# davide-coccomini/MINTIME-Multi-Identity-size-iNvariant-TIMEsformer-for-Video-Deepfake-Detection

Hardware: AMD Instinct MI355X
Metric: clips/sec (8-frame, 2-identity, 224^2 crops) fwd+bwd (higher is better)
Workload: dtype f32; 1 GPU; config 3: EfficientNet-B0 + SizeInvariantTimeSformer(dim 512, depth 9, heads 8), B=32/GPU, 8 frames, 2 identities (identity-masked), 224x224 crops, random-init seeded weights (restored before every step), train-mode BN + drop-connect 0.2, step = fwd + BCE loss + bwd + SGD(lr .01, wd 1e-4); global_batch=32, frames=8, parallelism=dp1

## Files before the change

include/mintime_hip.h:

```cpp
#ifndef MINTIME_HIP_H
#define MINTIME_HIP_H
#include <stdint.h>
#ifdef __cplusplus
extern "C" {
#endif

#define MT_VERSION 123

int mt_version(void);
const char* mt_last_error(void);

int mt_set_deterministic(int on);
int mt_get_deterministic(void);
int mt_det_release(void* stream);
int mt_det_bn_sums(const float* x, const float* z, const float* mean_invstd, int64_t rows, int C, int mode, double* stats, void* stream);

typedef struct { int gin, gout, off; } mt_rowmap;

enum { MT_OP_NT = 0,
       MT_OP_NN = 1,
       MT_OP_TN = 2 };

enum { MT_PRO_NONE = 0, MT_PRO_BN_SWISH_GATE = 1, MT_PRO_BN_SWISH = 2, MT_PRO_AFFINE = 3,
       MT_PRO_BN_BWD = 4,
// ... 48 lines not shown

int mt_bn_bwd_apply_planes(const float* du, const float* z, const float* kabc, void* planes, int rows, int C, void* stream);

typedef struct {
  int op;
  int epilogue;
  int M, N, K;
  const void* a_planes;
  const void* b_planes;
  float* C; int64_t ldc;
  const float* bias;
  const float* R; int64_t ldr;
  float* C2; int64_t ldc2;
  int n_half;
  float* col_sum;
  void* c_planes;
  int split_k;
  void* sk_workspace;
  int64_t sk_workspace_bytes;
  double* stats; int stats_slots;
} mt_gemm_planes_desc;

int mt_gemm_planes(const mt_gemm_planes_desc* d, void* stream);

int mt_mul_planes(const float* x, const float* m, void* planes, float* out, int rows, int cols, void* stream);
int mt_mul_add(const float* y, const float* m, const float* r, float* out, int64_t n, void* stream);
int mt_geglu_bwd(const float* dh, const float* m, const float* u, void* du_planes, float* du, int rows, int n_half, void* stream);
int64_t mt_gemm_planes_workspace_bytes(void);
int mt_gemm_planes_set_persist(int blocks_per_cu);


int mt_layernorm_fwd(const float* x, const float* gamma, const float* beta, float* y, float* stats,
                     int rows, int dim, float eps, void* y_planes, void* stream);

int mt_embed_fwd(float* x, const float* cls, const float* pos_emb, const float* size_emb,
                 const int64_t* positions, const int32_t* sizes, int B, int F, int n, int dim, int pos_rows, int size_rows,
                 int* err_flag, void* stream);

int mt_attn_fwd(const float* qkv, float* out, float* cls_att, const uint8_t* mask, const uint8_t* ident,
                int B, int H, int F, int n, int mode, float scale, void* out_planes, void* stream);

int mt_head_fwd(const float* x, const float* gamma, const float* beta, const float* w, const float* bias,
                float* logits, int B, int N, int dim, int classes, float eps, void* stream);


int mt_stem_conv_fwd(const void* x, int x_is_u8, const float* w, float* z, double* stats, int slots, int N, int H, int W,
// ... 256 lines not shown
```

mintime-multi-identity-size-invariant-timesformer-for-video-deepfake-detection_amd/csrc/gemm_planes.hip:

```cpp
#include "../../include/mintime_hip.h"
#include "common.hpp"
#include "gemm_planes_launch.hpp"
#include "gemm_geometry.hpp"
#include "det.hpp"
#include <string.h>

using namespace mt;

namespace {

__device__ __forceinline__ void to_blk_block(const float* __restrict__ src, int64_t ld, int R, int C, const PlaneRef& o, int rb, int cb, int lane) {
  const int r = rb * 32 + (lane >> 1), c = cb * 16 + (lane & 1) * 8;
  float x[8] = {0.f, 0.f, 0.f, 0.f, 0.f, 0.f, 0.f, 0.f};
  if (r < R) {
    const float* s = src + (int64_t)r * ld + c;
    if (c + 8 <= C && ((ld & 3) == 0) && (((uintptr_t)src & 15) == 0)) {
      const float4 u = *reinterpret_cast<const float4*>(s), v = *reinterpret_cast<const float4*>(s + 4);
      x[0] = u.x; x[1] = u.y; x[2] = u.z; x[3] = u.w; x[4] = v.x; x[5] = v.y; x[6] = v.z; x[7] = v.w;
    } else {
#pragma unroll
      for (int e = 0; e < 8; ++e) if (c + e < C) x[e] = s[e];
    }
  }
  planes_store8(o, r, c, x);
// ... 89 lines not shown
  const int cb16 = (cols + 15) >> 4, rp = (rows + 31) & ~31;
  const PlaneRef o{reinterpret_cast<__bf16*>(planes), (int64_t)rp * cb16 * 16, cb16, rp};
  hipLaunchKernelGGL(split_planes_blk_kernel, dim3((cb16 + 3) / 4, rp / 32), dim3(256), 0, (hipStream_t)stream, src, ld, rows, cols, o);
  return check_launch("mt_split_planes_blk");
}

extern "C" int mt_bn_bwd_apply_planes(const float* du, const float* z, const float* kabc, void* planes, int rows, int C, void* stream) {
  if (!du || !z || !kabc || !planes || rows <= 0 || C <= 0) return fail(MT_ERR_ARG, "mt_bn_bwd_apply_planes: bad arguments");
  if ((C & 3) || (((uintptr_t)du | (uintptr_t)z | (uintptr_t)kabc | (uintptr_t)planes) & 15))
    return fail(MT_ERR_ARG, "mt_bn_bwd_apply_planes: C %% 4 == 0 and 16-byte alignment");
  const int cb16 = (C + 15) >> 4, rp = (rows + 31) & ~31;
  const PlaneRef o{reinterpret_cast<__bf16*>(planes), (int64_t)rp * cb16 * 16, cb16, rp};
  hipLaunchKernelGGL(bn_bwd_apply_planes_kernel, dim3((cb16 + 3) / 4, rp / 32), dim3(256), 0, (hipStream_t)stream, du, z, kabc, rows, C, o);
  return check_launch("mt_bn_bwd_apply_planes");
}

extern "C" int mt_split_planes_blk_multi(const void* items, int count, int64_t total_blocks, void* stream) {
  if (!items || count <= 0 || total_blocks <= 0) return fail(MT_ERR_ARG, "mt_split_planes_blk_multi: bad arguments");
  hipLaunchKernelGGL(split_planes_blk_multi_kernel, dim3((unsigned)((total_blocks + 3) / 4)), dim3(256), 0, (hipStream_t)stream,
                     reinterpret_cast<const SplitItem*>(items), count, total_blocks);
  return check_launch("mt_split_planes_blk_multi");
}

static int gemm_planes_impl(const mt_gemm_planes_desc* d, void* stream) {
  if (!d || !d->a_planes || !d->b_planes) return fail(MT_ERR_ARG, "mt_gemm_planes: null operand planes");
  if (d->M <= 0 || d->N <= 0 || d->K <= 0) return fail(MT_ERR_ARG, "mt_gemm_planes: bad shape %d %d %d", d->M, d->N, d->K);
  if (((uintptr_t)d->a_planes & 15) || ((uintptr_t)d->b_planes & 15) || ((uintptr_t)d->c_planes & 15))
    return fail(MT_ERR_ARG, "mt_gemm_planes: planes must be 16-byte aligned");
  const int op = d->op, epi = d->epilogue;
  const bool cpl = d->c_planes != nullptr;
  if (!d->C && !cpl) return fail(MT_ERR_ARG, "mt_gemm_planes: no output");
  if (cpl && epi != MT_EPI_GEGLU && epi != MT_EPI_GEGLU_BWD) return fail(MT_ERR_UNSUPPORTED, "mt_gemm_planes: plane output only from the GEGLU pair");
  if (epi == MT_EPI_BIAS_RES && !d->R) return fail(MT_ERR_ARG, "mt_gemm_planes: BIAS_RES needs R");
  if (epi == MT_EPI_GEGLU && (d->n_half * 2 != d->N || (d->n_half & 63))) return fail(MT_ERR_ARG, "mt_gemm_planes GEGLU: N must be 2*n_half, n_half %% 64 == 0");
  if (epi == MT_EPI_GEGLU_BWD && (!d->C2 || d->n_half != d->N || (d->n_half & 31)))
    return fail(MT_ERR_ARG, "mt_gemm_planes GEGLU_BWD: needs C2, n_half == N and n_half %% 32 == 0");
  hipStream_t s = (hipStream_t)stream;
  const bool high = matmul_precision() == MT_PRECISION_HIGH;
  const int np = high ? 2 : 3;
  auto launch = [&](int skm, const GemmArgs& ga, dim3 g) {
    return high ? launch_planes_high(op, epi, cpl, skm, ga, g, s) : launch_planes_form<3>(op, epi, cpl, skm, ga, g, s);
  };

  const int a_rows = op == MT_OP_TN ? d->K : d->M, a_cols = op == MT_OP_TN ? d->M : d->K;
  const int b_rows = op == MT_OP_NT ? d->N : d->K, b_cols = op == MT_OP_NT ? d->K : d->N;
  GemmArgs a;
  memset(&a, 0, sizeof(a));
  a.C = d->C; a.M = d->M; a.N = d->N; a.K = d->K; a.ldc = d->ldc;
  a.a_planes = d->a_planes; a.a_pstride = mt_planes_elems(a_rows, a_cols); a.lda = (a_cols + 15) >> 4;
  a.b_planes = d->b_planes; a.b_pstride = mt_planes_elems(b_rows, b_cols); a.ldb = (b_cols + 15) >> 4;
  if (6 * a.a_pstride > 0xFFFFFFFFll || 6 * a.b_pstride > 0xFFFFFFFFll)
    return fail(MT_ERR_UNSUPPORTED, "mt_gemm_planes: an operand's planes span %lld bytes (> 4 GB: 32-bit DMA offsets); use mt_gemm for it (lib.planes_fit)",
                (long long)(6 * (a.a_pstride > a.b_pstride ? a.a_pstride : a.b_pstride)));
  a.bias = d->bias; a.R = d->R; a.ldr = d->ldr; a.C2 = d->C2; a.ldc2 = d->ldc2; a.n_half = d->n_half; a.col_sum = d->col_sum;
  a.hw = 1; a.stats_slots = d->stats_slots != 0 ? d->stats_slots : 1; a.stats = d->stats; a.b_hw = 1; a.e_hw = 1;
  if (epi == MT_EPI_STATS && !d->stats) return fail(MT_ERR_ARG, "mt_gemm_planes: STATS needs stats");
  if (epi == MT_EPI_GEGLU_BWD)
    if (int rc = det_gemm_colsum_setup(a.det, d->M, d->n_half, d->col_sum, s)) return rc;
  if (cpl) {
    const int c_cols = epi == MT_EPI_GEGLU ? d->n_half : 2 * d->n_half;
    a.c_planes = d->c_planes; a.c_pstride = mt_planes_elems(d->M, c_cols); a.ldcp = (c_cols + 15) >> 4;
  }

  const TileGrid tg = tile_grid(d->M, d->N, 128, 128, (int64_t)128 * d->K * 2 * np);
  const int m_tiles = tg.m_tiles, n_tiles = tg.n_tiles;
  if (op == MT_OP_TN) {
    if (epi != MT_EPI_ATOMIC) return fail(MT_ERR_UNSUPPORTED, "mt_gemm_planes TN: ATOMIC epilogue only (C pre-zeroed)");
    static const int target = env_int("MT_WGRAD_BLOCKS", 640);
    const SplitK sk = split_k_ranges(d->K, m_tiles * n_tiles, d->split_k, target, 16, K_XCD);
    a.k_chunk = sk.k_chunk; a.xcd_k = sk.xcd_k;
    if (int rc = det_gemm_setup(a.C, a.ldc, a.det_slab, d->M, d->N, sk.ranges, false, s)) return rc;
    return launch(0, a, dim3(m_tiles * n_tiles, sk.grid_y, 1));
  }
  dim3 grid(tg.grid_x, 1, 1);
  a.group_n = tg.group_n;
  static const int prio = env_int("MT_PLANES_MAIN_PRIO", 0);
  a.wave_prio = prio;
  bool sk = false;
  if (d->sk_workspace && d->sk_workspace_bytes >= mt_gemm_planes_workspace_bytes() && !((uintptr_t)d->sk_workspace & 255)) {
    int g = cu_count() * 2 / 8 * 8;
    if (g > kSkMaxGrid) g = kSkMaxGrid;
    const int64_t units = (int64_t)m_tiles * n_tiles * (((d->K + 15) / 16 + 1) / 2);
    if (g >= 8 && units >= (int64_t)g * 2 && units < (1ll << 30)) {
      sk = true;
      grid = dim3((unsigned)g, 1, 1);
      a.sk_on = 1;
      a.sk_flags = reinterpret_cast<int*>(d->sk_workspace);
      a.sk_ws = reinterpret_cast<float*>(reinterpret_cast<char*>(d->sk_workspace) + kSkFlagBytes);
    }
  }
  if (!sk && !cpl && (epi == MT_EPI_STORE || epi == MT_EPI_BIAS_RES)) {
    const int per_cu = persist_blocks();
    const int g = cu_count() * per_cu / 8 * 8;
    if (per_cu > 0 && g >= 8 && m_tiles * n_tiles > g) {
      const dim3 pg((unsigned)g, 1, 1);
      const bool nt_store = op == MT_OP_NT && epi == MT_EPI_STORE, nt_bias_res = op == MT_OP_NT && epi == MT_EPI_BIAS_RES;
      const bool nn_store = op == MT_OP_NN && epi == MT_EPI_STORE;
      if (nt_store || nt_bias_res || nn_store) return launch(2, a, pg);
    }
  }
  return launch(sk ? 1 : 0, a, grid);
}

extern "C" int mt_gemm_planes(const mt_gemm_planes_desc* d, void* stream) {
  const int rc = gemm_planes_impl(d, stream);
  if (rc) { (void)mt::det_gemm_finish(nullptr, false); return rc; }
  return mt::det_gemm_finish((hipStream_t)stream, true);
}
```

mintime-multi-identity-size-invariant-timesformer-for-video-deepfake-detection_amd/csrc/gemm_planes.hpp:

```cpp
#pragma once
#include "gemm_split.hpp"
#include "planes.hpp"

#ifndef MT_PLANES_ABLATE
#define MT_PLANES_ABLATE 0
#endif
#ifndef MT_PLANES_EPI_ABLATE
#define MT_PLANES_EPI_ABLATE 0
#endif
#ifndef MT_PLANES_PRIO
#define MT_PLANES_PRIO 0
#endif

namespace mt {

typedef short s16x4_t __attribute__((ext_vector_type(4)));
enum : int { BAL_NONE = 0, BAL_PAIR = 1, BAL_PHASE = 2 };

__device__ __forceinline__ void lds_dma16_s(const void* sbase, unsigned voff, unsigned lds_byte_addr) {
  unsigned keep;
  asm volatile("s_mov_b32 %0, m0\n\ts_mov_b32 m0, %3\n\ts_nop 0\n\tglobal_load_lds_dwordx4 %1, %2\n\ts_mov_b32 m0, %0"
               : "=&s"(keep) : "v"(voff), "s"(sbase), "s"(lds_byte_addr) : "memory");
}

// ... 90 lines not shown
        if (MT_PLANES_EPI_ABLATE & 4) { if (da[3] + dg[5] == 123.456f) p.col_sum[0] = 1.f; }
        else if (n0 + wn * TN * 32 + j * 32 < p.N) {
          planes_emit_tile(da, wl, o, mw + i * 32, n0 + wn * TN * 32 + j * 32, p.M, lane);
          planes_emit_tile(dg, wl, o, mw + i * 32, p.n_half + n0 + wn * TN * 32 + j * 32, p.M, lane);
        }
      }
      if (p.col_sum && !(MT_PLANES_EPI_ABLATE & 16)) {
        float t1 = s1[j], t2 = s2[j];
        t1 += __shfl_xor(t1, 32);
        t2 += __shfl_xor(t2, 32);
        if (lane < 32 && nok) {
          if (p.det.vals) {
            const int rk = mw >> 5;
            det_put(p.det, n >> 5, rk, n & 31, t1);
            det_put(p.det, (p.n_half + n) >> 5, rk, n & 31, t2);
            if (rk == 0 && (n & 31) == 0) { det_base(p.det, n >> 5, n); det_base(p.det, (p.n_half + n) >> 5, p.n_half + n); }
          } else {
            atomicAdd(p.col_sum + n, t1);
            atomicAdd(p.col_sum + p.n_half + n, t2);
          }
        }
      }
    }
  }
}

template <int BM, int BN>
__device__ __forceinline__ void sk_tile_coords(const GemmArgs& p, int t, int& mt_, int& nt_) {
  const int n_tiles = (p.N + BN - 1) / BN, m_tiles = (p.M + BM - 1) / BM;
  if (p.group_n > 0) {
    const int q = m_tiles >> 3, r = m_tiles & 7;
    int xcd = 0, base = 0;
    for (; xcd < 7; ++xcd) {
      const int cnt = (q + (xcd < r ? 1 : 0)) * n_tiles;
      if (t < base + cnt) break;
      base += cnt;
    }
    const int rows = q + (xcd < r ? 1 : 0);
    const int row0 = xcd < r ? xcd * (q + 1) : r * (q + 1) + (xcd - r) * q;
    const int idx = t - base;
    const int per_group = rows * p.group_n;
    const int g = idx / per_group;
    const int rem = idx - g * per_group;
    const int groups = (n_tiles + p.group_n - 1) / p.group_n;
    const int gw = (g == groups - 1) ? n_tiles - g * p.group_n : p.group_n;
    const int ml = rem / gw;
// ... 271 lines not shown
#pragma unroll
        for (int j = 0; j < TN; ++j) asm volatile("" : "+v"(acc[i][j]));
    }
  };

  auto epilogue = [&](int mt_, int nt_, int split_idx = -1) {
    if (MT_PLANES_ABLATE & 8) {
      float sacc = 0.f;
#pragma unroll
      for (int i = 0; i < TM; ++i)
#pragma unroll
        for (int j = 0; j < TN; ++j)
#pragma unroll
          for (int r = 0; r < 16; ++r) sacc += acc[i][j][r];
      if (sacc == 123.456f) p.C[0] = sacc;
      return;
    }
    int m0e = mt_ * BM, n0e = nt_ * BN, lane_e = lane;
    asm volatile("" : "+s"(m0e), "+s"(n0e), "+v"(lane_e));
    if constexpr (CPL) {
      static_assert(!CPL || STAGES * STAGE >= NW * 32 * 36 * 4, "the plane epilogue's LDS patches live in the main loop's stages");
      __syncthreads();
      planes_epilogue<TM, TN, EPI>(p, acc, m0e, n0e, wm, wn, lane_e, reinterpret_cast<float*>(smem_pl) + wave * (32 * 36));
    } else {
      gemm_epilogue<TM, TN, EPI>(p, acc, m0e, n0e, wm, wn, lane_e, split_idx);
    }
  };

  if (p.wave_prio == 1) __builtin_amdgcn_s_setprio(1);
  else if (p.wave_prio == 2) __builtin_amdgcn_s_setprio(2);
  else if (p.wave_prio == 3) __builtin_amdgcn_s_setprio(3);
  if (MT_PLANES_PRIO == 1) {
    const unsigned hwid = __builtin_amdgcn_s_getreg((4 << 0) | (0 << 6) | (3 << 11));
    if (__builtin_amdgcn_readfirstlane(hwid) & 1) __builtin_amdgcn_s_setprio(1);
  } else if (MT_PLANES_PRIO == 2) {
    if ((blockIdx.x >> 8) & 1) __builtin_amdgcn_s_setprio(1);
  }

  if constexpr (PS) {
    const int Q = gridDim.x >> 3, xcd = blockIdx.x & 7, q = blockIdx.x >> 3;
    const int n_tiles = (p.N + BN - 1) / BN, m_tiles = (p.M + BM - 1) / BM;
    int base = 0, cnt;
    if (p.group_n > 0) {
      const int qq = m_tiles >> 3, rr = m_tiles & 7;
      for (int i = 0; i < xcd; ++i) base += (qq + (i < rr ? 1 : 0)) * n_tiles;
      cnt = (qq + (xcd < rr ? 1 : 0)) * n_tiles;
// ... 212 lines not shown
```

mintime-multi-identity-size-invariant-timesformer-for-video-deepfake-detection_amd/csrc/gemm_planes_launch.hpp:

```cpp
#pragma once
#include "../../include/mintime_hip.h"
#include "common.hpp"
#include "gemm_planes.hpp"

#ifndef MT_PLANES_HIGH_STAGES
#define MT_PLANES_HIGH_STAGES 3
#endif

namespace mt {

template <int NP, bool AKM, bool BKM, int EPI, int BAL, bool CPL, int SK = 0>
int launch_planes(const GemmArgs& a, dim3 grid, hipStream_t s) {
  constexpr int ST = (NP == 2 && SK != 2) ? MT_PLANES_HIGH_STAGES : 2;
  auto k = gemm_planes_kernel<2, 2, 2, 2, AKM, BKM, EPI, ST, BAL == BAL_PAIR ? 2 : 3, BAL, CPL, SK, NP>;
  constexpr size_t lds = (size_t)ST * NP * (128 + 128) * 32;
  {
    hipError_t e = ensure_dynamic_lds(reinterpret_cast<const void*>(k), lds);
    if (e != hipSuccess) return fail(MT_ERR_LAUNCH, "mt_gemm_planes: cannot reserve %zu B of LDS: %s", lds, hipGetErrorString(e));
  }
  hipLaunchKernelGGL(k, grid, dim3(256), lds, s, a);
  return check_launch("mt_gemm_planes");
}

template <int NP>
int launch_planes_form(int op, int epi, bool cpl, int skm, const GemmArgs& a, dim3 grid, hipStream_t s) {
  if (op == MT_OP_TN && epi == MT_EPI_ATOMIC) return launch_planes<NP, true, true, EPI_ATOMIC, BAL_NONE, false, 0>(a, grid, s);
  if (skm == 2 && !cpl) {
    if (op == MT_OP_NT && epi == MT_EPI_STORE) return launch_planes<NP, false, false, EPI_STORE, BAL_PAIR, false, 2>(a, grid, s);
    if (op == MT_OP_NT && epi == MT_EPI_BIAS_RES) return launch_planes<NP, false, false, EPI_BIAS_RES, BAL_PAIR, false, 2>(a, grid, s);
    if (op == MT_OP_NN && epi == MT_EPI_STORE) return launch_planes<NP, false, true, EPI_STORE, BAL_PAIR, false, 2>(a, grid, s);
  }
  if (skm == 0 || skm == 1) {
#define PL_COMBO(OP, BKM_, EPI_, CPL_)                                                               \
  if (op == OP && epi == EPI_ && cpl == CPL_)                                                        \
    return skm ? launch_planes<NP, false, BKM_, EPI_, BAL_PAIR, CPL_, 1>(a, grid, s)                 \
               : launch_planes<NP, false, BKM_, EPI_, BAL_PAIR, CPL_, 0>(a, grid, s);
    PL_COMBO(MT_OP_NT, false, EPI_STORE, false)
    PL_COMBO(MT_OP_NT, false, EPI_BIAS_RES, false)
    PL_COMBO(MT_OP_NT, false, EPI_STATS, false)
    PL_COMBO(MT_OP_NT, false, EPI_GEGLU, false)
    PL_COMBO(MT_OP_NT, false, EPI_GEGLU, true)
    PL_COMBO(MT_OP_NN, true, EPI_STORE, false)
    PL_COMBO(MT_OP_NN, true, EPI_BIAS_RES, false)
    PL_COMBO(MT_OP_NN, true, EPI_GEGLU_BWD, false)
    PL_COMBO(MT_OP_NN, true, EPI_GEGLU_BWD, true)
#undef PL_COMBO
  }
  return fail(MT_ERR_UNSUPPORTED, "mt_gemm_planes: unsupported op / epilogue %d / %d", op, epi);
}

int launch_planes_high(int op, int epi, bool cpl, int skm, const GemmArgs& a, dim3 grid, hipStream_t s);

}
```

mintime-multi-identity-size-invariant-timesformer-for-video-deepfake-detection_amd/effnet_backward.py:

```python
import torch

from . import arch
from . import lib as L
from .effnet_engine import SLOTS, STREAM_ROWS, _StatsPool
from .lib import _new


FUSED_DW = __import__("os").environ.get("MT_DW_FUSED", "3")


def _splits(rows):
    return max(1, min(64, rows // 1024))


LAST_RUN = {"blocks_run": 0, "wgrad_launches": 0, "stem_run": False}


def effnet_backward(model, params, saved, shape, training, dfeat, need_dx, need_dparams, keep_saved=False, plan=None):
    lib = L.get()
    dev = dfeat.device
    N, H, W = shape
    blocks = model._blocks
    P = list(params)
    pos = 3
# ... 17 lines not shown
    if any(need[:3]):
        lowest = -1
    if need_dx:
        lowest = -1
        need_below = [True] * len(blocks)
        if W > 512:
            raise NotImplementedError("gradient w.r.t. the input crops: mt_stem_conv_dgrad takes crops of at most 512 columns")
    def runs_dw(bi):
        s, ix = blocks[bi].spec, bidx[bi]
        return need[ix["d"]] or need_below[bi] or (s.has_expand and any(need[ix["e"]:ix["e"] + 3]))
    odd = [b.spec.idx for bi, b in enumerate(blocks) if bi >= lowest and b.spec.s == 2 and b.spec.hin % 2 and runs_dw(bi)]
    if odd:
        raise NotImplementedError(f"EfficientNet backward for {H} x {W} crops: the stride-2 depthwise layers of blocks {odd} see odd "
                                  "sizes, which mt_dwconv_bwd does not take")
    grads, flat_grads = L.zero_grads(list(params), with_flat=True)
    dx = None
    run = {"blocks_run": 0, "wgrad_launches": 0, "stem_run": False}
    total_c = arch.STEM_COUT + arch.HEAD_COUT + sum((b.spec.cexp if b.spec.has_expand else 0) + b.spec.cexp + b.spec.cout
                                                    for b in blocks)
    tr = 1 if training else 0
    side = L.SideStream(dev, hold=True)

    det = L.deterministic()
    pool = _StatsPool(dev, total_c, det)
    slots = -SLOTS if det else SLOTS
    fused_dw = "0" if det else FUSED_DW

    def bn_finalize(bnctx, sums, gidx_gamma, d=None, z=None, rows=0):
        kabc = _new(dev, 3, bnctx.C)
        L.mt.bn_bwd_finalize(sums, slots, bnctx.count, P[gidx_gamma], bnctx.mean_invstd, kabc, grads[gidx_gamma], grads[gidx_gamma + 1],
                             bnctx.C, tr)
        return kabc

    def act_bwd(din, z, bnctx, dout, rows, hw, act, gate=None, dpool=None, rowscale=None):
        sums = pool.take(bnctx.C)
        L.mt.bn_act_bwd(din, z, bnctx.scale, bnctx.shift, bnctx.mean_invstd, gate, dpool, rowscale, dout, sums, slots, rows, bnctx.C, hw,
                        act)
        return sums

    def conv1x1_bwd(du, z, kabc, w, x_in, rows, cout, cin, gw_idx, need_dx_in, res=None, b_pro=None, pl=None):
        if pl is not None:
            dz_p = L.planes_empty(rows, cout, dev)
            L.mt.bn_bwd_apply_planes(du, z, kabc, dz_p, rows, cout)
            wdone = False
            if need[gw_idx] and pl.get("x_p") is not None:
                run["wgrad_launches"] += 1
                side.launch(lambda: L.gemm_planes(L.OP_TN, dz_p, pl["x_p"], cout, cin, rows, Cout=grads[gw_idx].view(cout, cin), ldc=cin,
                                                  epilogue=L.EPI_ATOMIC), reads=(dz_p, pl["x_p"]))
                wdone = True
            dx_in = None
            if need_dx_in:
                dx_in = _new(dev, rows, cin)
                if res is not None:
                    L.gemm_planes(L.OP_NN, dz_p, pl["w_p"], rows, cin, cout, Cout=dx_in, ldc=cin, epilogue=L.EPI_BIAS_RES, R=res, ldr=cin)
                else:
                    L.gemm_planes(L.OP_NN, dz_p, pl["w_p"], rows, cin, cout, Cout=dx_in, ldc=cin)
            if wdone or not need[gw_idx]:
                return dx_in
            need_dx_in, keep_dx = False, dx_in
        else:
            keep_dx = None
        kw = {}
        if b_pro is not None:
            kw = dict(b_prologue=L.BPRO_BN_SWISH_GATE, b_scale=b_pro[0], b_shift=b_pro[1], b_gate=b_pro[2], b_hw=b_pro[3])
        reads = (du, z, x_in, kabc) + (tuple(b_pro[:3]) if b_pro is not None else ())
        if (not det and b_pro is None and need[gw_idx] and need_dx_in and rows >= STREAM_ROWS
                and lib.mt_conv1x1_bwd_fused_supported(cout, cin)):
            run["wgrad_launches"] += 1
            dx_in = _new(dev, rows, cin)
            L.mt.conv1x1_bwd_fused(du, kabc, x_in, w, res, dx_in, grads[gw_idx], rows, cout, cin)
            return dx_in
        if not need[gw_idx]:
            pass
        elif rows >= STREAM_ROWS and not det and lib.mt_conv1x1_wgrad_supported(cout, cin):
            run["wgrad_launches"] += 1
            bp = b_pro if b_pro is not None else (None, None, None, 1)
            side.launch(lambda: L.mt.conv1x1_wgrad(du, z, kabc, x_in, bp[0], bp[1], bp[2], bp[3], grads[gw_idx], rows, cout, cin),
# ... 26 lines not shown
    M = N * s_last.hout * s_last.hout
    du_h = _new(dev, M, arch.HEAD_COUT)
    sums = act_bwd(dfeat, hd["z"], hd["bn"], du_h, M, 1, 1)
    kabc = bn_finalize(hd["bn"], sums, ih + 1, du_h, hd["z"], M)
    dy = conv1x1_bwd(du_h, hd["z"], kabc, P[ih], hd["y_in"], M, arch.HEAD_COUT, arch.HEAD_CIN, ih, lowest < len(blocks),
                     pl=dict(w_p=hd["w_p"], x_p=hd["y_p"]) if hd.get("w_p") is not None else None)
    del du_h

    for bi in reversed(range(len(blocks))):
        if bi < lowest:
            break
        run["blocks_run"] += 1
        blk, rec, ix = blocks[bi], saved["blocks"][bi], bidx[bi]
        s = rec["spec"]
        M_in, M_out = N * s.hin * s.hin, N * s.hout * s.hout
        hw = s.hout * s.hout
        dc = rec["dc"]
        dyb = _new(dev, M_out, s.cout) if dc is not None else None
        sums = act_bwd(dy, rec["z_p"], rec["bn_p"], dyb, M_out, hw, 0, rowscale=dc)
        dsrc = dyb if dc is not None else dy
        kabc_p = bn_finalize(rec["bn_p"], sums, ix["p"] + 1, dsrc, rec["z_p"], M_out)
        bn_d = rec["bn_d"]
        b_pro = (bn_d.scale, bn_d.shift, rec["gate"], hw)
        dgate, dpre2, dpooled = _new(dev, N, s.cexp), _new(dev, N, s.cexp), _new(dev, N, s.cexp)
        dhid = _new(dev, N, s.cse)
        se_scr = _new(dev, lib.mt_se_scratch_floats(N, s.cexp, s.cse))
        se = ix["se"]
        def se_part(parts, _da=None, _rec=rec, _bn=bn_d, _se=se, _s=s, _dg=dgate, _dp=dpre2, _dh=dhid, _dpo=dpooled, _hw=hw, _scr=se_scr):
            L.mt.se_bwd(_da, _rec["z_d"], _bn.scale, _bn.shift, _rec["gate"], _rec["hidden"], _rec["pooled"], P[_se], P[_se + 2], _dg, _dp,
                        _dh, _dpo, grads[_se], grads[_se + 1], grads[_se + 2], grads[_se + 3], N, _hw, _s.cexp, _s.cse, parts, _scr)
        if not det and M_out >= STREAM_ROWS and lib.mt_se_stage_fused_supported(s.cout, s.cexp, hw):
            conv1x1_bwd(dsrc, rec["z_p"], kabc_p, P[ix["p"]], rec["z_d"], M_out, s.cout, s.cexp, ix["p"], False, b_pro=b_pro)
            def stage(mode, dg, g_, dpo, mi, out, st_):
                L.mt.se_stage_fused(dsrc, rec["z_p"], kabc_p, P[ix["p"]], rec["z_d"], bn_d.scale, bn_d.shift, mode, dg, g_, dpo, mi, out,
                                    st_, slots, M_out, s.cout, s.cexp, hw)
            L.zero_(dgate)
            stage(0, dgate, None, None, None, None, None)
            se_part(4)
            if any(need[se:se + 4]):
                run["wgrad_launches"] += 1
                side.launch(lambda: se_part(2), reads=(dpre2, dhid, rec["hidden"], rec["pooled"]))
            da = _new(dev, M_out, s.cexp)
            sums = pool.take(s.cexp)
            stage(1, None, rec["gate"], dpooled, bn_d.mean_invstd, da, sums)
        else:
            da = conv1x1_bwd(dsrc, rec["z_p"], kabc_p, P[ix["p"]], rec["z_d"], M_out, s.cout, s.cexp, ix["p"], True, b_pro=b_pro,
                             pl=dict(w_p=rec["wp_p"], x_p=rec["a_p"]) if rec.get("wp_p") is not None else None)
            se_part(1, da)
            if any(need[se:se + 4]):
                run["wgrad_launches"] += 1
                side.launch(lambda: se_part(2), reads=(dpre2, dhid, rec["hidden"], rec["pooled"]))
            sums = act_bwd(da, rec["z_d"], bn_d, da, M_out, hw, 1, gate=rec["gate"], dpool=dpooled)
        kabc_d = bn_finalize(bn_d, sums, ix["d"] + 1, da, rec["z_d"], M_out)
        in_bn = rec["dw_bn"]
        du_in = _new(dev, M_in, s.cexp)
        sums_in = pool.take(s.cexp)
        def dw_part(parts, _da=da, _rec=rec, _kabc=kabc_d, _bn=in_bn, _du_in=du_in, _sums=sums_in, _s=s, _ix=ix):
            L.mt.dwconv_bwd(_da, _rec["z_d"], _kabc, P[_ix["d"]], _rec["dw_in"], _bn.scale, _bn.shift, _bn.mean_invstd, _du_in, _sums,
                            slots, grads[_ix["d"]], N, _s.hin, _s.hin, _s.cexp, _s.k, _s.s, parts, 1, None, None)
        need_du_in = need_below[bi] or (s.has_expand and any(need[ix["e"]:ix["e"] + 3]))
        dw_bytes = 4.0 * s.cexp * (2 * M_out + 2 * M_in)
        if not need_du_in or not need[ix["d"]]:
            if need[ix["d"]]:
                run["wgrad_launches"] += 1
                side.launch(lambda: dw_part(1), reads=(da, rec["z_d"], kabc_d, rec["dw_in"], in_bn.scale, in_bn.shift))
            if need_du_in:
                L.timed("dwconv_dgrad", lambda: dw_part(2), dw_bytes)
        elif fused_dw == "1" or (fused_dw == "3" and s.k == 3):
            run["wgrad_launches"] += 1
            L.timed("dwconv_dgrad", lambda: dw_part(3), dw_bytes)
        else:
# ... 35 lines not shown
```

mintime-multi-identity-size-invariant-timesformer-for-video-deepfake-detection_amd/effnet_engine.py:

```python
import threading

import torch

from . import arch
from . import lib as L
from . import plans
from .lib import _new

SLOTS = 32
STREAM_ROWS = 100000
EF_PLANES_EXPAND_HW, EF_PLANES_PROJECT_HW = 14, 7


def param_list(model):
    ps = [model._conv_stem.weight, model._bn0.weight, model._bn0.bias]
    for blk in model._blocks:
        if blk.spec.has_expand:
            ps += [blk._expand_conv.weight, blk._bn0.weight, blk._bn0.bias]
        ps += [blk._depthwise_conv.weight, blk._bn1.weight, blk._bn1.bias, blk._se_reduce.weight, blk._se_reduce.bias,
               blk._se_expand.weight, blk._se_expand.bias, blk._project_conv.weight, blk._bn2.weight, blk._bn2.bias]
    ps += [model._conv_head.weight, model._bn1.weight, model._bn1.bias]
    return ps


class _BNCtx:

    def __init__(self, dev, C, training, stats_pool):
        self.C = C
        self.scale, self.shift = _new(dev, C), _new(dev, C)
        self.mean_invstd = _new(dev, 2, C)
        self.stats = stats_pool.take(C) if training else None
        self.count = 0.0


class _StatsPool:

    def __init__(self, dev, total_channels, det=False):
        self.limbs = 2 if det else 1
        self.buf = L.zeros(total_channels * 2 * SLOTS * self.limbs, torch.float64, dev)
        self.off = 0

    def take(self, C):
        n = 2 * SLOTS * C * self.limbs
        v = self.buf[self.off:self.off + n]
        self.off += n
        return v


def _finalize(bn_mod, ctx, count, training, gamma, beta, slots=SLOTS, st=None):
    ctx.count = float(count)
    L.mt.bn_finalize(ctx.stats, slots, float(count), gamma, beta, bn_mod.running_mean, bn_mod.running_var, ctx.scale, ctx.shift,
                     ctx.mean_invstd, ctx.C, bn_mod.eps, bn_mod.momentum, 1 if training else 0, L.stream_ptr() if st is None else st)
    if training:
        _track(bn_mod.num_batches_tracked)


_TLS = threading.local()


def _track(counter):
    if not hasattr(_TLS, "tracked"):
        _TLS.tracked = []
    _TLS.tracked.append(counter)


def planes_scope(model, N):
    on = L.gemm_split_enabled()
    blocks = model._blocks
# ... 262 lines not shown
```

mintime-multi-identity-size-invariant-timesformer-for-video-deepfake-detection_amd/lib.py:

```python
import ctypes as C
import os
import subprocess
import threading

import torch

_HERE = os.path.dirname(os.path.abspath(__file__))
CSRC = os.path.join(_HERE, "csrc")
LIB_PATH = os.environ.get("MT_LIB") or os.path.join(CSRC, "libmintime_hip.so")

_lib = None
i64 = C.c_int64


class f32p(C.c_void_p):
    """`float*` / `const float*` of the header: a pointer slot that takes fp32 tensors only (passed as a plain pointer)."""


class RowMap(C.Structure):
    _fields_ = [("gin", C.c_int), ("gout", C.c_int), ("off", C.c_int)]


class Conv3dDesc(C.Structure):
    _fields_ = [(n, C.c_int) for n in ("N", "T", "H", "W", "C", "To", "Ho", "Wo", "K", "kt", "kh", "kw", "st", "sh", "sw", "pt", "ph",
# ... 26 lines not shown

class GemmPlanesDesc(C.Structure):
    _fields_ = [("op", C.c_int), ("epilogue", C.c_int), ("M", C.c_int), ("N", C.c_int), ("K", C.c_int),
                ("a_planes", C.c_void_p), ("b_planes", C.c_void_p), ("C", C.c_void_p), ("ldc", i64),
                ("bias", C.c_void_p), ("R", C.c_void_p), ("ldr", i64), ("C2", C.c_void_p), ("ldc2", i64),
                ("n_half", C.c_int), ("col_sum", C.c_void_p), ("c_planes", C.c_void_p), ("split_k", C.c_int),
                ("sk_workspace", C.c_void_p), ("sk_workspace_bytes", i64), ("stats", C.c_void_p), ("stats_slots", C.c_int)]


OP_NT, OP_NN, OP_TN = 0, 1, 2
PRO_NONE, PRO_BN_SWISH_GATE, PRO_BN_SWISH, PRO_AFFINE, PRO_BN_BWD, PRO_IM2COL = 0, 1, 2, 3, 4, 5
BPRO_NONE, BPRO_BN_SWISH_GATE, BPRO_IM2COL = 0, 1, 2
EPI_STORE, EPI_BIAS_RES, EPI_GEGLU, EPI_STATS, EPI_ATOMIC, EPI_GEGLU_BWD, EPI_ACCUM, EPI_SE_RED, EPI_ACT_BWD = 0, 1, 2, 3, 4, 5, 6, 7, 8

LAUNCHES = {
    "mt_det_release": [C.c_void_p],
    "mt_det_bn_sums": [f32p, f32p, f32p, i64, C.c_int, C.c_int, C.c_void_p, C.c_void_p],
    "mt_gemm": [C.POINTER(GemmDesc), C.c_void_p],
    "mt_split_planes": [f32p, C.c_void_p, i64, C.c_void_p],
    "mt_split_planes_blk": [f32p, i64, C.c_int, C.c_int, C.c_void_p, C.c_void_p],
    "mt_split_planes_blk_multi": [C.c_void_p, C.c_int, i64, C.c_void_p],
    "mt_bn_bwd_apply_planes": [f32p, f32p, f32p, C.c_void_p, C.c_int, C.c_int, C.c_void_p],
    "mt_gemm_planes": [C.POINTER(GemmPlanesDesc), C.c_void_p],
    "mt_mul_planes": [f32p, f32p, C.c_void_p, f32p, C.c_int, C.c_int, C.c_void_p],
    "mt_mul_add": [f32p] * 4 + [i64, C.c_void_p],
    "mt_geglu_bwd": [f32p, f32p, f32p, C.c_void_p, f32p, C.c_int, C.c_int, C.c_void_p],
    "mt_layernorm_fwd": [f32p] * 5 + [C.c_int, C.c_int, C.c_float, C.c_void_p, C.c_void_p],
    "mt_embed_fwd": [f32p] * 4 + [C.c_void_p, C.c_void_p] + [C.c_int] * 6 + [C.c_void_p, C.c_void_p],
    "mt_attn_fwd": [f32p, f32p, f32p, C.c_void_p, C.c_void_p] + [C.c_int] * 5 + [C.c_float, C.c_void_p, C.c_void_p],
    "mt_head_fwd": [f32p] * 6 + [C.c_int] * 4 + [C.c_float, C.c_void_p],
    "mt_stem_conv_fwd": [C.c_void_p, C.c_int, f32p, f32p, C.c_void_p] + [C.c_int] * 4 + [C.c_void_p],
    "mt_stem_conv_fwd_valid": [C.c_void_p, C.c_int, f32p, f32p, C.c_void_p] + [C.c_int] * 4 + [C.c_void_p],
    "mt_dwconv_fwd": [f32p] * 5 + [C.c_void_p] + [C.c_int] * 8 + [C.c_void_p],
    "mt_dwconv_fwd_planes": [f32p] * 4 + [C.c_void_p] + [C.c_int] * 7 + [C.c_void_p],
    "mt_bn_finalize": [C.c_void_p, C.c_int, C.c_double] + [f32p] * 7 + [C.c_int, C.c_float, C.c_float, C.c_int, C.c_void_p],
    "mt_se_pool_fwd": [f32p] * 4 + [C.c_int] * 4 + [C.c_void_p],
    "mt_se_gate_fwd": [f32p, C.c_int] + [f32p] * 7 + [C.c_int, C.c_int, C.c_int, C.c_void_p],
    "mt_bn_act_fwd": [f32p] * 5 + [i64, C.c_int, C.c_int, f32p, C.c_int, C.c_void_p],
    "mt_attn_aggregate": [f32p, f32p, f32p, C.c_int, C.c_int, C.c_int, C.c_float, C.c_void_p],
    "mt_build_clip_inputs": [C.c_void_p] * 8 + [C.c_int] * 5 + [C.c_void_p],
    "mt_layernorm_bwd": [f32p] * 7 + [C.c_int, C.c_int, C.c_int, f32p, C.c_int, f32p, C.c_void_p],
    "mt_layernorm_bwd_rows": [f32p] * 6 + [C.c_int, C.c_int, C.c_void_p, C.c_void_p],
    "mt_layernorm_bwd_cols": [f32p] * 7 + [C.c_int, C.c_int, C.c_int, C.c_void_p],
    "mt_layernorm_bwd_rows_sums": [f32p] * 6 + [C.c_int, C.c_int, C.c_void_p, f32p, C.c_int, C.c_void_p],
    "mt_layernorm_bwd_rows_sums_sparse": [f32p] * 6 + [C.c_int, C.c_int, C.c_int, C.c_void_p, f32p, C.c_int, C.c_void_p],
    "mt_layernorm_bwd_cols_reduce": [f32p, C.c_int, C.c_int, f32p, f32p, f32p, C.c_void_p],
# ... 76 lines not shown
    "mt_memset_async": [C.c_void_p, C.c_int, i64, C.c_void_p],
    "mt_copy_async": [C.c_void_p, C.c_void_p, i64, C.c_void_p],
}
QUERIES = {
    "mt_version": [],
    "mt_last_error": [],
    "mt_set_deterministic": [C.c_int],
    "mt_get_deterministic": [],
    "mt_gemm_set_split": [C.c_int],
    "mt_gemm_get_split": [],
    "mt_gemm_set_precision": [C.c_int],
    "mt_gemm_get_precision": [],
    "mt_planes_elems": [C.c_int, C.c_int],
    "mt_gemm_planes_workspace_bytes": [],
    "mt_gemm_planes_set_persist": [C.c_int],
    "mt_se_pool_parts": [C.c_int, C.c_int, C.c_int],
    "mt_layernorm_bwd_rows_blocks": [C.c_int],
    "mt_se_scratch_floats": [C.c_int, C.c_int, C.c_int],
    "mt_conv1x1_rows_supported": [C.c_int, C.c_int, C.c_int],
    "mt_conv1x1_wgrad_supported": [C.c_int, C.c_int],
    "mt_conv1x1_wgrad_wide_supported": [C.c_int, C.c_int],
    "mt_conv1x1_bwd_fused_supported": [C.c_int, C.c_int],
    "mt_se_stage_fused_supported": [C.c_int, C.c_int, C.c_int],
    "mt_conv3d_part_floats": [C.c_void_p],
    "mt_conv3d_wgrad_splits": [C.c_void_p],
    "mt_sf_bn_bwd_part_floats": [i64, C.c_int],
    "mt_plan_create": [C.POINTER(C.c_void_p)],
    "mt_plan_destroy": [C.c_void_p],
    "mt_plan_record_begin": [C.c_void_p],
    "mt_plan_record_end": [C.c_void_p],
    "mt_plan_size": [C.c_void_p],
    "mt_plan_tag": [C.c_int, C.c_double],
    "mt_plan_fork": [C.c_void_p, C.c_void_p],
    "mt_plan_run": [C.c_void_p, C.c_uint],
    "mt_plan_probe_read": [C.c_void_p, C.c_int, C.POINTER(C.c_int), C.POINTER(C.c_double), C.POINTER(C.c_double)],
}
PROTOTYPES = {**QUERIES, **LAUNCHES}
_RESTYPES = {"mt_last_error": C.c_char_p, "mt_planes_elems": C.c_int64, "mt_gemm_planes_workspace_bytes": C.c_int64,
             "mt_conv3d_part_floats": C.c_int64, "mt_sf_bn_bwd_part_floats": C.c_int64}


class MintimeHipError(RuntimeError):
    pass


def build(verbose: bool = False):
# ... 181 lines not shown

_SK_WORKSPACES = {}


def streamk_workspace(device=None):
    st = torch.cuda.current_stream(device)
    key = (st.device.index, st.cuda_stream)
    ws = _SK_WORKSPACES.get(key)
    if ws is None:
        if torch.cuda.is_current_stream_capturing():
            return None
        n = get().mt_gemm_planes_workspace_bytes()
        ws = torch.zeros(n, dtype=torch.uint8, device=st.device)
        _SK_WORKSPACES[key] = ws
    return ws


def planes_fit(rows: int, cols: int) -> bool:
    rp, cp = (rows + 31) // 32 * 32, (cols + 15) // 16 * 16
    return 6 * rp * cp <= 0xFFFFFFFF


def gemm_planes(op, a_planes, b_planes, M, N, K, Cout=None, ldc=0, epilogue=EPI_STORE, bias=None, R=None, ldr=0, C2=None, ldc2=0,
                n_half=0, col_sum=None, c_planes=None, split_k=0, streamk=None, stats=None, stats_slots=0):
    d = GemmPlanesDesc()
    if streamk is None:
        streamk = os.environ.get("MT_PLANES_STREAMK", "0") != "0"
    if streamk and op != OP_TN:
        ws = streamk_workspace(a_planes.device)
        if ws is not None:
            d.sk_workspace, d.sk_workspace_bytes = ptr(ws), ws.numel()
    d.op, d.epilogue, d.M, d.N, d.K = op, epilogue, M, N, K
    d.a_planes, d.b_planes, d.C, d.ldc = ptr(a_planes), ptr(b_planes), ptr(Cout), ldc
    d.bias, d.R, d.ldr, d.C2, d.ldc2 = ptr(bias), ptr(R), ldr, ptr(C2), ldc2
    d.n_half, d.col_sum, d.c_planes, d.split_k = n_half, ptr(col_sum), ptr(c_planes), split_k
    d.stats, d.stats_slots = ptr(stats), stats_slots
    if recording() is not None:
        if op == OP_TN:
            tag_next(TAG_WGRAD, 2.0 * M * N * K)
        elif epilogue == EPI_GEGLU:
            tag_next(TAG_FF1, 2.0 * M * N * K)
    prof = PROFILE
    if prof is not None:
        for pr in prof:
            if "match_planes" in pr and pr["match_planes"](d):
                e0, e1 = torch.cuda.Event(enable_timing=True), torch.cuda.Event(enable_timing=True)
                e0.record()
                mt.gemm_planes(d)
                e1.record()
                pr["events"].append((e0, e1, 2.0 * M * N * K))
                return
    mt.gemm_planes(d)


def gemm_split_enabled() -> bool:
    return bool(get().mt_gemm_get_split())


def check(rc, what):
# ... 274 lines not shown
```

Measured before the change: 733.2 clips/s.

## Fuse SE gate-gradient reduction into the projection dgrad GEMM epilogue

Adds an SE_RED epilogue to the planes GEMM. It computes the per-image, per-channel sum of da * swish(bn(z_d)) from the accumulators, reduces through LDS and atomically adds into dgate. The EfficientNet backward uses it when the projection dgrad runs on planes, and passes a different mode to se_part. dgate now comes from the pre-zeroed stats pool, which removes the separate zeroing. The aim is to skip a separate pass that rereads da and z_d for the SE backward. In exchange it adds fp32 atomics, so results become nondeterministic (it is disabled in deterministic mode), extra strided C2 loads in the epilogue, and no stream-K for these GEMMs.

```diff
diff --git a/include/mintime_hip.h b/include/mintime_hip.h
--- a/include/mintime_hip.h
+++ b/include/mintime_hip.h
@@ -94,6 +94,10 @@
 } mt_gemm_planes_desc;
 
 int mt_gemm_planes(const mt_gemm_planes_desc* d, void* stream);
+
+int mt_gemm_planes_se_red(const mt_gemm_planes_desc* d, const float* e_scale, const float* e_shift, int e_hw, float* dgate,
+                          void* stream);
+int mt_gemm_planes_se_red_supported(int M, int N, int K, int e_hw);
 
 int mt_mul_planes(const float* x, const float* m, void* planes, float* out, int rows, int cols, void* stream);
 int mt_mul_add(const float* y, const float* m, const float* r, float* out, int64_t n, void* stream);
diff --git a/mintime-multi-identity-size-invariant-timesformer-for-video-deepfake-detection_amd/csrc/gemm_planes.hip b/mintime-multi-identity-size-invariant-timesformer-for-video-deepfake-detection_amd/csrc/gemm_planes.hip
--- a/mintime-multi-identity-size-invariant-timesformer-for-video-deepfake-detection_amd/csrc/gemm_planes.hip
+++ b/mintime-multi-identity-size-invariant-timesformer-for-video-deepfake-detection_amd/csrc/gemm_planes.hip
@@ -135,7 +135,9 @@
   return check_launch("mt_split_planes_blk_multi");
 }
 
-static int gemm_planes_impl(const mt_gemm_planes_desc* d, void* stream) {
+struct SeRedArgs { const float* e_scale; const float* e_shift; int e_hw; float* dgate; };
+
+static int gemm_planes_impl(const mt_gemm_planes_desc* d, void* stream, const SeRedArgs* se = nullptr) {
   if (!d || !d->a_planes || !d->b_planes) return fail(MT_ERR_ARG, "mt_gemm_planes: null operand planes");
   if (d->M <= 0 || d->N <= 0 || d->K <= 0) return fail(MT_ERR_ARG, "mt_gemm_planes: bad shape %d %d %d", d->M, d->N, d->K);
   if (((uintptr_t)d->a_planes & 15) || ((uintptr_t)d->b_planes & 15) || ((uintptr_t)d->c_planes & 15))
@@ -145,6 +147,17 @@
   if (!d->C && !cpl) return fail(MT_ERR_ARG, "mt_gemm_planes: no output");
   if (cpl && epi != MT_EPI_GEGLU && epi != MT_EPI_GEGLU_BWD) return fail(MT_ERR_UNSUPPORTED, "mt_gemm_planes: plane output only from the GEGLU pair");
   if (epi == MT_EPI_BIAS_RES && !d->R) return fail(MT_ERR_ARG, "mt_gemm_planes: BIAS_RES needs R");
+  if ((epi == MT_EPI_SE_RED) != (se != nullptr)) return fail(MT_ERR_UNSUPPORTED, "mt_gemm_planes: SE_RED goes through mt_gemm_planes_se_red (and nothing else does)");
+  if (se) {
+    if (op != MT_OP_NN || cpl) return fail(MT_ERR_UNSUPPORTED, "mt_gemm_planes_se_red: op NN with fp32 output only");
+    if (!d->C || !d->C2 || !se->e_scale || !se->e_shift || !se->dgate) return fail(MT_ERR_ARG, "mt_gemm_planes_se_red: needs C (da), C2 (z_d), e_scale, e_shift and dgate");
+    if (d->bias) return fail(MT_ERR_ARG, "mt_gemm_planes_se_red: takes no bias");
+    if (se->e_hw <= 0 || d->M % se->e_hw) return fail(MT_ERR_ARG, "mt_gemm_planes_se_red: M must be a positive multiple of e_hw");
+    if (d->ldc < d->N || d->ldc2 < d->N) return fail(MT_ERR_ARG, "mt_gemm_planes_se_red: ldc, ldc2 >= N");
+    if (127 / se->e_hw + 2 > SE_RED_IMGS)
+      return fail(MT_ERR_UNSUPPORTED, "mt_gemm_planes_se_red: images of %d rows (a 128-row tile would touch more than %d)", se->e_hw, SE_RED_IMGS);
+    if (det_enabled()) return fail(MT_ERR_UNSUPPORTED, "mt_gemm_planes_se_red: fp32 atomics; deterministic mode keeps mt_gemm_planes + mt_se_bwd");
+  }
   if (epi == MT_EPI_GEGLU && (d->n_half * 2 != d->N || (d->n_half & 63))) return fail(MT_ERR_ARG, "mt_gemm_planes GEGLU: N must be 2*n_half, n_half %% 64 == 0");
   if (epi == MT_EPI_GEGLU_BWD && (!d->C2 || d->n_half != d->N || (d->n_half & 31)))
     return fail(MT_ERR_ARG, "mt_gemm_planes GEGLU_BWD: needs C2, n_half == N and n_half %% 32 == 0");
@@ -167,6 +180,7 @@
                 (long long)(6 * (a.a_pstride > a.b_pstride ? a.a_pstride : a.b_pstride)));
   a.bias = d->bias; a.R = d->R; a.ldr = d->ldr; a.C2 = d->C2; a.ldc2 = d->ldc2; a.n_half = d->n_half; a.col_sum = d->col_sum;
   a.hw = 1; a.stats_slots = d->stats_slots != 0 ? d->stats_slots : 1; a.stats = d->stats; a.b_hw = 1; a.e_hw = 1;
+  if (se) { a.e_scale = se->e_scale; a.e_shift = se->e_shift; a.e_hw = se->e_hw; a.col_sum = se->dgate; }
   if (epi == MT_EPI_STATS && !d->stats) return fail(MT_ERR_ARG, "mt_gemm_planes: STATS needs stats");
   if (epi == MT_EPI_GEGLU_BWD)
     if (int rc = det_gemm_colsum_setup(a.det, d->M, d->n_half, d->col_sum, s)) return rc;
@@ -190,6 +204,7 @@
   static const int prio = env_int("MT_PLANES_MAIN_PRIO", 0);
   a.wave_prio = prio;
   bool sk = false;
+  if (se) return launch(0, a, grid);
   if (d->sk_workspace && d->sk_workspace_bytes >= mt_gemm_planes_workspace_bytes() && !((uintptr_t)d->sk_workspace & 255)) {
     int g = cu_count() * 2 / 8 * 8;
     if (g > kSkMaxGrid) g = kSkMaxGrid;
@@ -215,6 +230,18 @@
   return launch(sk ? 1 : 0, a, grid);
 }
 
+extern "C" int mt_gemm_planes_se_red_supported(int M, int N, int K, int e_hw) {
+  if (M <= 0 || N <= 0 || K <= 0 || e_hw <= 0 || M % e_hw) return 0;
+  if (127 / e_hw + 2 > SE_RED_IMGS) return 0;
+  return det_enabled() ? 0 : 1;
+}
+
+extern "C" int mt_gemm_planes_se_red(const mt_gemm_planes_desc* d, const float* e_scale, const float* e_shift, int e_hw, float* dgate,
+                                     void* stream) {
+  const SeRedArgs se{e_scale, e_shift, e_hw, dgate};
+  return gemm_planes_impl(d, stream, &se);
+}
+
 extern "C" int mt_gemm_planes(const mt_gemm_planes_desc* d, void* stream) {
   const int rc = gemm_planes_impl(d, stream);
   if (rc) { (void)mt::det_gemm_finish(nullptr, false); return rc; }
diff --git a/mintime-multi-identity-size-invariant-timesformer-for-video-deepfake-detection_amd/csrc/gemm_planes.hpp b/mintime-multi-identity-size-invariant-timesformer-for-video-deepfake-detection_amd/csrc/gemm_planes.hpp
--- a/mintime-multi-identity-size-invariant-timesformer-for-video-deepfake-detection_amd/csrc/gemm_planes.hpp
+++ b/mintime-multi-identity-size-invariant-timesformer-for-video-deepfake-detection_amd/csrc/gemm_planes.hpp
@@ -136,6 +136,65 @@
         }
       }
     }
+  }
+}
+
+constexpr int SE_RED_IMGS = 8;
+
+template <int WAVES_M, int TM, int TN, int BN, int NT>
+__device__ __forceinline__ void planes_se_red(const GemmArgs& p, const f32x16 (&acc)[TM][TN], int m0, int n0, int wm, int wn, int lane,
+                                              int tid, float* red) {
+  constexpr int BM = WAVES_M * TM * 32;
+  constexpr int CELLS = WAVES_M * 2 * SE_RED_IMGS * BN;
+  for (int i = tid * 4; i < CELLS; i += NT * 4) *reinterpret_cast<float4*>(red + i) = make_float4(0.f, 0.f, 0.f, 0.f);
+  __syncthreads();
+  const int col_l = lane & 31, hf = lane >> 5;
+  const int mfirst = m0 + wm * TM * 32 + hf * 4;
+  const int img0 = m0 / p.e_hw;
+  float* mine = red + (wm * 2 + hf) * (SE_RED_IMGS * BN);
+#pragma unroll
+  for (int j = 0; j < TN; ++j) {
+    const int cb = wn * TN * 32 + j * 32 + col_l;
+    const bool nok = n0 + cb < p.N;
+    const int nn = nok ? n0 + cb : p.N - 1;
+    const float esc = p.e_scale[nn], esh = p.e_shift[nn];
+    int img = mfirst / p.e_hw;
+    int rem = mfirst - img * p.e_hw;
+    int prev = 0;
+    float run = 0.f;
+    auto put = [&]() { if (run != 0.f && img - img0 < SE_RED_IMGS) mine[(img - img0) * BN + cb] = run; };
+#pragma unroll
+    for (int i = 0; i < TM; ++i) {
+      float zv[16];
+#pragma unroll
+      for (int r = 0; r < 16; ++r) {
+        const int m = mfirst + i * 32 + (r & 3) + 8 * (r >> 2);
+        zv[r] = p.C2[(int64_t)min(m, p.M - 1) * p.ldc2 + nn];
+      }
+#pragma unroll
+      for (int r = 0; r < 16; ++r) {
+        const int dr = i * 32 + (r & 3) + 8 * (r >> 2);
+        rem += dr - prev;
+        prev = dr;
+        if (rem >= p.e_hw) {
+          put();
+          run = 0.f;
+          do { rem -= p.e_hw; ++img; } while (rem >= p.e_hw);
+        }
+        if (mfirst + dr < p.M && nok) run = fmaf(acc[i][j][r], swishf_(fmaf(zv[r], esc, esh)), run);
+      }
+    }
+    put();
+  }
+  __syncthreads();
+  const int img_last = (min(m0 + BM, p.M) - 1) / p.e_hw;
+  for (int i = tid; i < SE_RED_IMGS * BN; i += NT) {
+    const int sl = i / BN, c = i - sl * BN;
+    if (img0 + sl > img_last || n0 + c >= p.N) continue;
+    float v = 0.f;
+#pragma unroll
+    for (int w = 0; w < WAVES_M * 2; ++w) v += red[w * (SE_RED_IMGS * BN) + i];
+    if (v != 0.f) atomicAdd(p.col_sum + (int64_t)(img0 + sl) * p.N + n0 + c, v);
   }
 }
 
@@ -453,6 +512,12 @@
       static_assert(!CPL || STAGES * STAGE >= NW * 32 * 36 * 4, "the plane epilogue's LDS patches live in the main loop's stages");
       __syncthreads();
       planes_epilogue<TM, TN, EPI>(p, acc, m0e, n0e, wm, wn, lane_e, reinterpret_cast<float*>(smem_pl) + wave * (32 * 36));
+    } else if constexpr (EPI == EPI_SE_RED) {
+      static_assert(EPI != EPI_SE_RED || (SKM == 0 && STAGES * STAGE >= WAVES_M * 2 * SE_RED_IMGS * BN * 4),
+                    "SE_RED: one block per tile; its cells live in the main loop's stages");
+      __syncthreads();
+      planes_se_red<WAVES_M, TM, TN, BN, NW * 64>(p, acc, m0e, n0e, wm, wn, lane_e, tid, reinterpret_cast<float*>(smem_pl));
+      gemm_epilogue<TM, TN, EPI_STORE>(p, acc, m0e, n0e, wm, wn, lane_e, split_idx);
     } else {
       gemm_epilogue<TM, TN, EPI>(p, acc, m0e, n0e, wm, wn, lane_e, split_idx);
     }
diff --git a/mintime-multi-identity-size-invariant-timesformer-for-video-deepfake-detection_amd/csrc/gemm_planes_launch.hpp b/mintime-multi-identity-size-invariant-timesformer-for-video-deepfake-detection_amd/csrc/gemm_planes_launch.hpp
--- a/mintime-multi-identity-size-invariant-timesformer-for-video-deepfake-detection_amd/csrc/gemm_planes_launch.hpp
+++ b/mintime-multi-identity-size-invariant-timesformer-for-video-deepfake-detection_amd/csrc/gemm_planes_launch.hpp
@@ -30,6 +30,7 @@
     if (op == MT_OP_NT && epi == MT_EPI_BIAS_RES) return launch_planes<NP, false, false, EPI_BIAS_RES, BAL_PAIR, false, 2>(a, grid, s);
     if (op == MT_OP_NN && epi == MT_EPI_STORE) return launch_planes<NP, false, true, EPI_STORE, BAL_PAIR, false, 2>(a, grid, s);
   }
+  if (op == MT_OP_NN && epi == MT_EPI_SE_RED && !cpl && skm == 0) return launch_planes<NP, false, true, EPI_SE_RED, BAL_PAIR, false, 0>(a, grid, s);
   if (skm == 0 || skm == 1) {
 #define PL_COMBO(OP, BKM_, EPI_, CPL_)                                                               \
   if (op == OP && epi == EPI_ && cpl == CPL_)                                                        \
diff --git a/mintime-multi-identity-size-invariant-timesformer-for-video-deepfake-detection_amd/effnet_backward.py b/mintime-multi-identity-size-invariant-timesformer-for-video-deepfake-detection_amd/effnet_backward.py
--- a/mintime-multi-identity-size-invariant-timesformer-for-video-deepfake-detection_amd/effnet_backward.py
+++ b/mintime-multi-identity-size-invariant-timesformer-for-video-deepfake-detection_amd/effnet_backward.py
@@ -63,7 +63,7 @@
     side = L.SideStream(dev, hold=True)
 
     det = L.deterministic()
-    pool = _StatsPool(dev, total_c, det)
+    pool = _StatsPool(dev, total_c, det, extra_f32=sum(N * b.spec.cexp for b in blocks))
     slots = -SLOTS if det else SLOTS
     fused_dw = "0" if det else FUSED_DW
 
@@ -79,7 +79,7 @@
                         act)
         return sums
 
-    def conv1x1_bwd(du, z, kabc, w, x_in, rows, cout, cin, gw_idx, need_dx_in, res=None, b_pro=None, pl=None):
+    def conv1x1_bwd(du, z, kabc, w, x_in, rows, cout, cin, gw_idx, need_dx_in, res=None, b_pro=None, pl=None, se_red=None):
         if pl is not None:
             dz_p = L.planes_empty(rows, cout, dev)
             L.mt.bn_bwd_apply_planes(du, z, kabc, dz_p, rows, cout)
@@ -94,6 +94,9 @@
                 dx_in = _new(dev, rows, cin)
                 if res is not None:
                     L.gemm_planes(L.OP_NN, dz_p, pl["w_p"], rows, cin, cout, Cout=dx_in, ldc=cin, epilogue=L.EPI_BIAS_RES, R=res, ldr=cin)
+                elif se_red is not None:
+                    L.gemm_planes(L.OP_NN, dz_p, pl["w_p"], rows, cin, cout, Cout=dx_in, ldc=cin, epilogue=L.EPI_SE_RED, C2=se_red[0],
+                                  ldc2=cin, se_red=se_red[1:])
                 else:
                     L.gemm_planes(L.OP_NN, dz_p, pl["w_p"], rows, cin, cout, Cout=dx_in, ldc=cin)
             if wdone or not need[gw_idx]:
@@ -166,7 +169,7 @@
         kabc_p = bn_finalize(rec["bn_p"], sums, ix["p"] + 1, dsrc, rec["z_p"], M_out)
         bn_d = rec["bn_d"]
         b_pro = (bn_d.scale, bn_d.shift, rec["gate"], hw)
-        dgate, dpre2, dpooled = _new(dev, N, s.cexp), _new(dev, N, s.cexp), _new(dev, N, s.cexp)
+        dgate, dpre2, dpooled = pool.take_f32(N, s.cexp), _new(dev, N, s.cexp), _new(dev, N, s.cexp)
         dhid = _new(dev, N, s.cse)
         se_scr = _new(dev, lib.mt_se_scratch_floats(N, s.cexp, s.cse))
         se = ix["se"]
@@ -178,7 +181,6 @@
             def stage(mode, dg, g_, dpo, mi, out, st_):
                 L.mt.se_stage_fused(dsrc, rec["z_p"], kabc_p, P[ix["p"]], rec["z_d"], bn_d.scale, bn_d.shift, mode, dg, g_, dpo, mi, out,
                                     st_, slots, M_out, s.cout, s.cexp, hw)
-            L.zero_(dgate)
             stage(0, dgate, None, None, None, None, None)
             se_part(4)
             if any(need[se:se + 4]):
@@ -188,9 +190,12 @@
             sums = pool.take(s.cexp)
             stage(1, None, rec["gate"], dpooled, bn_d.mean_invstd, da, sums)
         else:
+            on_planes = rec.get("wp_p") is not None
+            fused_red = on_planes and bool(lib.mt_gemm_planes_se_red_supported(M_out, s.cexp, s.cout, hw))
             da = conv1x1_bwd(dsrc, rec["z_p"], kabc_p, P[ix["p"]], rec["z_d"], M_out, s.cout, s.cexp, ix["p"], True, b_pro=b_pro,
-                             pl=dict(w_p=rec["wp_p"], x_p=rec["a_p"]) if rec.get("wp_p") is not None else None)
-            se_part(1, da)
+                             pl=dict(w_p=rec["wp_p"], x_p=rec["a_p"]) if on_planes else None,
+                             se_red=(rec["z_d"], bn_d.scale, bn_d.shift, hw, dgate) if fused_red else None)
+            se_part(4 if fused_red else 1, da)
             if any(need[se:se + 4]):
                 run["wgrad_launches"] += 1
                 side.launch(lambda: se_part(2), reads=(dpre2, dhid, rec["hidden"], rec["pooled"]))
diff --git a/mintime-multi-identity-size-invariant-timesformer-for-video-deepfake-detection_amd/effnet_engine.py b/mintime-multi-identity-size-invariant-timesformer-for-video-deepfake-detection_amd/effnet_engine.py
--- a/mintime-multi-identity-size-invariant-timesformer-for-video-deepfake-detection_amd/effnet_engine.py
+++ b/mintime-multi-identity-size-invariant-timesformer-for-video-deepfake-detection_amd/effnet_engine.py
@@ -35,15 +35,25 @@
 
 class _StatsPool:
 
-    def __init__(self, dev, total_channels, det=False):
+    def __init__(self, dev, total_channels, det=False, extra_f32=0):
         self.limbs = 2 if det else 1
-        self.buf = L.zeros(total_channels * 2 * SLOTS * self.limbs, torch.float64, dev)
+        self.buf = L.zeros(total_channels * 2 * SLOTS * self.limbs + (extra_f32 + 1) // 2, torch.float64, dev)
         self.off = 0
+        self.f32 = self.buf[total_channels * 2 * SLOTS * self.limbs:].view(torch.float32)
+        self.off_f32 = 0
 
     def take(self, C):
         n = 2 * SLOTS * C * self.limbs
         v = self.buf[self.off:self.off + n]
         self.off += n
+        return v
+
+    def take_f32(self, *shape):
+        n = 1
+        for d in shape:
+            n *= d
+        v = self.f32[self.off_f32:self.off_f32 + n].view(*shape)
+        self.off_f32 += (n + 3) // 4 * 4
         return v
 
 
diff --git a/mintime-multi-identity-size-invariant-timesformer-for-video-deepfake-detection_amd/lib.py b/mintime-multi-identity-size-invariant-timesformer-for-video-deepfake-detection_amd/lib.py
--- a/mintime-multi-identity-size-invariant-timesformer-for-video-deepfake-detection_amd/lib.py
+++ b/mintime-multi-identity-size-invariant-timesformer-for-video-deepfake-detection_amd/lib.py
@@ -72,6 +72,7 @@
     "mt_split_planes_blk_multi": [C.c_void_p, C.c_int, i64, C.c_void_p],
     "mt_bn_bwd_apply_planes": [f32p, f32p, f32p, C.c_void_p, C.c_int, C.c_int, C.c_void_p],
     "mt_gemm_planes": [C.POINTER(GemmPlanesDesc), C.c_void_p],
+    "mt_gemm_planes_se_red": [C.POINTER(GemmPlanesDesc), f32p, f32p, C.c_int, f32p, C.c_void_p],
     "mt_mul_planes": [f32p, f32p, C.c_void_p, f32p, C.c_int, C.c_int, C.c_void_p],
     "mt_mul_add": [f32p] * 4 + [i64, C.c_void_p],
     "mt_geglu_bwd": [f32p, f32p, f32p, C.c_void_p, f32p, C.c_int, C.c_int, C.c_void_p],
@@ -194,6 +195,7 @@
     "mt_conv1x1_wgrad_wide_supported": [C.c_int, C.c_int],
     "mt_conv1x1_bwd_fused_supported": [C.c_int, C.c_int],
     "mt_se_stage_fused_supported": [C.c_int, C.c_int, C.c_int],
+    "mt_gemm_planes_se_red_supported": [C.c_int, C.c_int, C.c_int, C.c_int],
     "mt_conv3d_part_floats": [C.c_void_p],
     "mt_conv3d_wgrad_splits": [C.c_void_p],
     "mt_sf_bn_bwd_part_floats": [i64, C.c_int],
@@ -421,8 +423,10 @@
 
 
 def gemm_planes(op, a_planes, b_planes, M, N, K, Cout=None, ldc=0, epilogue=EPI_STORE, bias=None, R=None, ldr=0, C2=None, ldc2=0,
-                n_half=0, col_sum=None, c_planes=None, split_k=0, streamk=None, stats=None, stats_slots=0):
+                n_half=0, col_sum=None, c_planes=None, split_k=0, streamk=None, stats=None, stats_slots=0, se_red=None):
     d = GemmPlanesDesc()
+    if se_red is not None:
+        streamk = False
     if streamk is None:
         streamk = os.environ.get("MT_PLANES_STREAMK", "0") != "0"
     if streamk and op != OP_TN:
@@ -434,6 +438,10 @@
     d.bias, d.R, d.ldr, d.C2, d.ldc2 = ptr(bias), ptr(R), ldr, ptr(C2), ldc2
     d.n_half, d.col_sum, d.c_planes, d.split_k = n_half, ptr(col_sum), ptr(c_planes), split_k
     d.stats, d.stats_slots = ptr(stats), stats_slots
+    if se_red is not None:
+        e_scale, e_shift, e_hw, dgate = se_red
+        mt.gemm_planes_se_red(d, e_scale, e_shift, e_hw, dgate)
+        return
     if recording() is not None:
         if op == OP_TN:
             tag_next(TAG_WGRAD, 2.0 * M * N * K)
```

Result: no change. 733.6 clips/s (median of 2 runs) (+0.0%).
